# kai-neumann/OrthoSfM

Hardware: AMD Instinct MI355X
Metric: image-pairs matched/sec + BA iterations/sec (N images, M tracks) at 1/2/4/8 GPU (higher is better)
Workload: dtype i8; 1 GPU; 50 orthographic images, 20000 SIFT features/img, exhaustive matching (1225 pairs, low-res gate + two-way + cross-check + lists; SURVEY 8d's unit of work: up to, not including, RANSAC-F -- the pass through RANSAC-F is `with_geometric_verification`); views=50, features_per_view=20000, pairs=1225

## Files before the change

orthosfm_amd/csrc/match_kernels.hip:

```cpp
#include <algorithm>

#include "match_kernels.h"

namespace osfm {


typedef int v4i __attribute__((ext_vector_type(4)));
typedef int v16i __attribute__((ext_vector_type(16)));


__device__ __forceinline__ int max3i(int a, int b, int c)
{
    int r;
    asm("v_max3_i32 %0, %1, %2, %3" : "=v"(r) : "v"(a), "v"(b), "v"(c));
    return r;
}
__device__ __forceinline__ int med3a(int a, int b, int c)
{
    int r;
    asm("v_med3_i32 %0, %1, %2, %3" : "=v"(r) : "v"(a), "v"(b), "v"(c));
    return r;
}

constexpr int kGroupTiles = 8;
constexpr int kPipeGroupTiles = 16;
constexpr int kPipeTileBits = 9;
constexpr int kValNone = -(1 << 28);

template <int V> struct IntC { static constexpr int value = V; };

__device__ __forceinline__ void store_colpart(ColPart *dst, const ColPart &v)
{
#ifdef OSFM_COLPART_PLAIN_STORE
    *dst = v;
#else
    __builtin_nontemporal_store(*reinterpret_cast<const unsigned long long *>(&v), reinterpret_cast<unsigned long long *>(dst));
#endif
}

template <int CH, bool MASKED, bool RAW, bool C0>
__device__ __forceinline__ void
tile_body(const MatchProblem &pd, int rb, int seg, RowPart *__restrict__ rowparts,
    ColPart *__restrict__ colparts, char *smem, const int8_t *__restrict__ zero_tile)
{
    static_assert(!C0 || RAW, "the correction-free form needs the raw row operand");
    constexpr int D = CH * 16;
    constexpr int KS = CH / 2;
    constexpr int RPB = 16 / CH;
    constexpr int TILE_BYTES = kTileCols * D;
    constexpr int CHUNKS = kTileCols * CH;
    constexpr int CPT = CHUNKS / 256;
    constexpr int BBUF_BYTES = 2 * TILE_BYTES > 16384 ? 2 * TILE_BYTES : 16384;
    constexpr int kRawShift = C0 ? kPipeTileBits : 7;
    constexpr int kCurNone = RAW ? -(1 << (30 - kRawShift)) : kKeyNone;
    static_assert(kSegCols / kTileCols <= (1 << 7), "tile index must fit the key");
    constexpr bool PIPE = C0;
    constexpr int NCHUNK = 2 * KS;
    constexpr int RPC = 16 / NCHUNK;
    constexpr int CPC = 16 / KS;

    char *bbuf = smem;
    int *corrbuf = reinterpret_cast<int *>(smem + BBUF_BYTES);
    ColPart *colbuf = reinterpret_cast<ColPart *>(smem + BBUF_BYTES + 2 * 64 * 4);
    int *rsecbuf = reinterpret_cast<int *>(smem + BBUF_BYTES + 2 * 64 * 4 + 8 * 4 * 64 * 8);

    const int n1 = pd.n1, n2 = pd.n2, n2stride = pd.n2stride;
    const int8_t *const Bbase = C0 ? pd.B_raw : pd.B;
    const int32_t *const corrBbase = pd.corrB;
    ColPart *const colout = colparts + pd.colpart_off + (int64_t)rb * pd.n2stride;
    const int tid = threadIdx.x;
    const int wave = tid >> 6, lane = tid & 63, lr = lane & 31, lh = lane >> 5;
    const int row0 = rb * kRowsPerBlock + wave * 64;
    const int gcode = wave * 2 + lh;

    const int8_t *Abase = pd.A;
    const int32_t *corrA = pd.corrA;
    int arow0 = row0;
    if (RAW) { Abase = pd.A_raw; corrA = pd.corrA_raw; }
    else if (!MASKED && rb >= pd.nrb_main) {
        Abase = pd.A_special; corrA = pd.corrA_special;
        arow0 = (rb - pd.nrb_main) * kRowsPerBlock + wave * 64;
    }
    v4i a[2][KS];
    v16i ra[2];
#pragma unroll
    for (int rf = 0; rf < 2; ++rf) {
        const int8_t *arow = Abase + (size_t)(arow0 + rf * 32 + lr) * D;
#pragma unroll
        for (int ks = 0; ks < KS; ++ks)
            a[rf][ks] = *reinterpret_cast<const v4i *>(arow + (ks * 2 + lh) * 16);
#pragma unroll
        for (int r = 0; r < 16; ++r)
            ra[rf][r] = C0 ? 0 : corrA[arow0 + rf * 32 + (r & 3) + 8 * (r >> 2) + 4 * lh];
    }
    const v16i zero16 = {0, 0, 0, 0, 0, 0, 0, 0, 0, 0, 0, 0, 0, 0, 0, 0};
    unsigned row_valid_bits = 0xffffffffu;
    if (MASKED) {
        row_valid_bits = 0;
#pragma unroll
        for (int fr = 0; fr < 32; ++fr) {
            const int row = row0 + (fr >> 4) * 32 + (fr & 3) + 8 * ((fr >> 2) & 3) + 4 * lh;
            row_valid_bits |= (row < n1 ? 1u : 0u) << fr;
        }
    }

    v16i rbest[2], rcur[2];
#pragma unroll
    for (int rf = 0; rf < 2; ++rf)
#pragma unroll
        for (int r = 0; r < 16; ++r) {
            rbest[rf][r] = kKeyNone; rcur[rf][r] = kCurNone;
            rsecbuf[(rf * 16 + r) * 256 + tid] = kKeyNone;
        }

    const int seg_cols = pd.seg_cols;
    const int col_begin = seg * seg_cols;
    const int col_lim = min(n2, col_begin + seg_cols);
    const int ntiles = (col_lim - col_begin + kTileCols - 1) / kTileCols;

    typedef __attribute__((address_space(3))) void lds_void;
    typedef const __attribute__((address_space(1))) void glb_void;
    const int wave_s = __builtin_amdgcn_readfirstlane(wave);
    unsigned lane_off[CPT];
#pragma unroll
    for (int c = 0; c < CPT; ++c) {
        const int q = (c * 4 + wave) * 64 + lane;
        const int col = q / CH;
        const int ch = (q % CH) ^ ((col / RPB) % CH);
        lane_off[c] = (unsigned)(col * D + ch * 16);
    }
    auto dma_wait = [&](bool store_behind = false) {
        if (!PIPE) return;
#ifndef OSFM_TILE_WAIT_ALL
        if (store_behind) { asm volatile("s_waitcnt vmcnt(1)" ::: "memory"); return; }
#endif
        asm volatile("s_waitcnt vmcnt(0)" ::: "memory");
    };
    auto stage_tile = [&](int t, int buf) {
        const int8_t *src = Bbase + (size_t)(col_begin + t * kTileCols) * D;
        if (PIPE && t >= ntiles) src = zero_tile;
#pragma unroll
        for (int c = 0; c < CPT; ++c) {
            const int q0 = (c * 4 + wave_s) * 64;
            if (PIPE) {
                static_assert(!PIPE || RAW, "the PIPE schedule must not contain compiler-managed m0 users");
                const unsigned lds_at = (unsigned)(uintptr_t)(bbuf + buf * TILE_BYTES + q0 * 16);
                asm volatile("s_mov_b32 m0, %2\n\tglobal_load_lds_dwordx4 %0, %1"
                             :: "v"(lane_off[c]), "s"(src), "s"(lds_at) : "memory");
            } else {
                __builtin_amdgcn_global_load_lds(
                    (glb_void *)(src + lane_off[c]),
                    (lds_void *)(uintptr_t)(bbuf + buf * TILE_BYTES + q0 * 16), 16, 0, 0);
            }
        }
        if (!RAW && wave_s == 0)
            __builtin_amdgcn_global_load_lds(
                (glb_void *)(corrBbase + col_begin + t * kTileCols + lane),
                (lds_void *)(uintptr_t)(corrbuf + buf * 64), 4, 0, 0);
    };

    v4i b[2][KS];
    int cb_next[2] = {0, 0};
    auto load_b = [&](int buf, int cf) {
        const int col = cf * 32 + lr;
        const int swz = (col / RPB) % CH;
#pragma unroll
        for (int ks = 0; ks < KS; ++ks)
            b[cf][ks] = *reinterpret_cast<const v4i *>(
                bbuf + buf * TILE_BYTES + col * D + (((ks * 2 + lh) ^ swz) * 16));
        if (!RAW) cb_next[cf] = corrbuf[buf * 64 + col];
    };

    int cbj[2] = {0, 0}, cjt[2] = {0, 0};
    bool col_valid[2] = {true, true};
    int g[2] = {kValNone, kValNone};

    v16i acc0[2], acc1[2];

    auto phase = [&](auto ph_c, auto cl_c, auto mg_c, auto rs_c, v16i (&cur)[2], v16i (&nxt)[2], int buf_next,
                     int tile0, int tm) {
        constexpr int PH = decltype(ph_c)::value;
        constexpr int CL = decltype(cl_c)::value;
        constexpr int RS = decltype(rs_c)::value;
        constexpr bool MG = decltype(mg_c)::value != 0;
        constexpr int OF = PH ^ 1;
        int sv = 0;
        ColPart cpm[4];
        if (CL >= 0) sv = rsecbuf[(OF * 16 + CL) * 256 + tid];
        if (MG) {
#pragma unroll
            for (int w = 0; w < 4; ++w) cpm[w] = colbuf[((tm & 7) * 4 + w) * 64 + lane];
        }
#pragma unroll
        for (int i = 0; i < NCHUNK; ++i) {
            const int cf = i / KS, ks = i % KS;
            if (ks == 0)
                nxt[cf] = __builtin_amdgcn_mfma_i32_32x32x32_i8(a[PH ^ 1][0], b[cf][0], C0 ? zero16 : ra[PH ^ 1], 0, 0, 0);
            else
                nxt[cf] = __builtin_amdgcn_mfma_i32_32x32x32_i8(a[PH ^ 1][ks], b[cf][ks], nxt[cf], 0, 0, 0);
            if (PH == 0 && i == KS - 1) load_b(buf_next, 0);
            if (PH == 1 && i == 0) {
                __builtin_amdgcn_sched_barrier(0);
                load_b(buf_next, 1);
            }

#pragma unroll
            for (int r = i * RPC; r < (i + 1) * RPC; ++r) {
                if (RAW) {
                    if (RS >= 0 && r == RS) rcur[PH][r] = max(cur[0][r], cur[1][r]);
                    else rcur[PH][r] = max(max(rcur[PH][r], cur[0][r]), cur[1][r]);
                } else {
                    int k0 = (int)(((unsigned)cur[0][r] << 8) + (unsigned)cjt[0]);
                    int k1 = (int)(((unsigned)cur[1][r] << 8) + (unsigned)cjt[1]);
                    if (MASKED) {
                        k0 = col_valid[0] ? k0 : kKeyNone;
                        k1 = col_valid[1] ? k1 : kKeyNone;
                    }
                    rcur[PH][r] = max3i(rcur[PH][r], k0, k1);
                }
            }
            {
                int x[CPC];
#pragma unroll
                for (int j = 0; j < CPC; ++j) {
                    x[j] = cur[cf][ks * CPC + j];
                    if (MASKED) x[j] = ((row_valid_bits >> (PH * 16 + ks * CPC + j)) & 1u) ? x[j] : kValNone;
                }
                int gg;
                if (PH == 0 && ks == 0) gg = max(x[0], x[1]);
                else gg = max(max(g[cf], x[0]), x[1]);
#pragma unroll
                for (int j = 2; j < CPC; j += 2) gg = max(max(gg, x[j]), x[j + 1]);
                asm volatile("" : "+v"(gg));
                g[cf] = gg;
            }
            if (CL >= 0 && i == 2) {
                const int r = CL;
                const int gk = (int)(((unsigned)rcur[OF][r] << kRawShift) | (unsigned)tile0);
                rsecbuf[(OF * 16 + r) * 256 + tid] = med3a(rbest[OF][r], sv, gk);
                rbest[OF][r] = max(rbest[OF][r], gk);
            }
            if (MG && (i == 2 || i == 3)) {
                if (i == 2) {
                    int k1 = cpm[0].key_best, k2 = cpm[0].key_second;
#pragma unroll
                    for (int w = 1; w < 4; ++w) {
                        k2 = max(max(min(k1, cpm[w].key_best), k2), cpm[w].key_second);
                        k1 = max(k1, cpm[w].key_best);
                    }
                    cpm[0].key_best = k1; cpm[0].key_second = k2;
                } else {
                    store_colpart(colout + col_begin + tm * kTileCols + lane, cpm[0]);
                }
            }
            __builtin_amdgcn_sched_barrier(0);
        }
    };

    stage_tile(0, 0);
    stage_tile(PIPE || ntiles > 1 ? 1 : 0, 1);
    dma_wait();
    __syncthreads();
    load_b(0, 0);
    load_b(0, 1);
#pragma unroll
    for (int cf = 0; cf < 2; ++cf) {
        acc0[cf] = __builtin_amdgcn_mfma_i32_32x32x32_i8(a[0][0], b[cf][0], C0 ? zero16 : ra[0], 0, 0, 0);
#pragma unroll
        for (int ks = 1; ks < KS; ++ks)
            acc0[cf] = __builtin_amdgcn_mfma_i32_32x32x32_i8(a[0][ks], b[cf][ks], acc0[cf], 0, 0, 0);
    }
    __syncthreads();

    auto tile_top = [&](int t) {
        stage_tile(PIPE ? t + 2 : min(t + 2, ntiles - 1), t & 1);
#pragma unroll
        for (int cf = 0; cf < 2; ++cf) {
            if (!RAW) {
                cbj[cf] = cb_next[cf];
                cjt[cf] = (int)(((unsigned)cbj[cf] << 8) + (unsigned)(t * 2 + cf));
                asm volatile("" : "+v"(cjt[cf]));
            }
            col_valid[cf] = (col_begin + t * kTileCols + cf * 32 + lr) < n2;
        }
    };
    auto tile_bottom = [&](int t, bool store_behind = false) {
        int kk[2];
#pragma unroll
        for (int cf = 0; cf < 2; ++cf) {
            kk[cf] = (int)((unsigned)(g[cf] + cbj[cf]) << 8) | gcode;
            if (MASKED) kk[cf] = g[cf] < -(1 << 27) ? kKeyNone : kk[cf];
        }
        const auto sw = __builtin_amdgcn_permlane32_swap((unsigned)kk[0], (unsigned)kk[1], false, false);
        const int x0 = (int)sw[0], x1 = (int)sw[1];
        ColPart cp;
        cp.key_best = max(x0, x1);
        cp.key_second = min(x0, x1);
        colbuf[((t & 7) * 4 + wave) * 64 + lane] = cp;
        dma_wait(store_behind);
        __syncthreads();
    };
    auto close_all = [&](auto first_tile) {
        int sv[2][16];
#pragma unroll
        for (int rf = 0; rf < 2; ++rf)
#pragma unroll
            for (int r = 0; r < 16; ++r) sv[rf][r] = rsecbuf[(rf * 16 + r) * 256 + tid];
#pragma unroll
        for (int rf = 0; rf < 2; ++rf)
#pragma unroll
            for (int r = 0; r < 16; ++r) {
                const int gk = RAW ? (int)(((unsigned)rcur[rf][r] << kRawShift) | (unsigned)first_tile(rf, r)) : rcur[rf][r];
                rsecbuf[(rf * 16 + r) * 256 + tid] = med3a(rbest[rf][r], sv[rf][r], gk);
                rbest[rf][r] = max(rbest[rf][r], gk);
                rcur[rf][r] = kCurNone;
            }
    };
    auto merge_tile = [&](int tm) {
        ColPart cp[4];
#pragma unroll
        for (int w = 0; w < 4; ++w) cp[w] = colbuf[((tm & 7) * 4 + w) * 64 + lane];
        int k1 = cp[0].key_best, k2 = cp[0].key_second;
#pragma unroll
        for (int w = 1; w < 4; ++w) {
            k2 = max(max(min(k1, cp[w].key_best), k2), cp[w].key_second);
            k1 = max(k1, cp[w].key_best);
        }
        const int col = col_begin + tm * kTileCols + lane;
        if (col < n2stride) {
            ColPart out;
            out.key_best = k1;
            out.key_second = k2;
            store_colpart(colout + col, out);
        }
    };

    int t = 0;
    if (PIPE) {
        static_assert(kPipeGroupTiles == 16, "the staggered schedule closes one of 16 slots per phase");
        auto cycle_tile = [&](auto u_c, int t0) {
            constexpr int u = decltype(u_c)::value;
            const int tt = t0 + u;
            tile_top(tt);
            const int bn = (tt & 1) ^ 1;
            const int tm = max(tt - 5, 0) + wave;
            phase(IntC<0>(), IntC<u>(), IntC<(u & 3) == 1 ? 1 : 0>(), IntC<(u + 15) & 15>(), acc0, acc1, bn,
                max(tt - 16, 0), tm);
            phase(IntC<1>(), IntC<u>(), IntC<0>(), IntC<u>(), acc1, acc0, bn, max(tt - 15, 0), 0);
            tile_bottom(tt, (u & 3) == 1);
        };
        const int tcyc = (ntiles + 15) & ~15;
        for (; t < tcyc; t += 16) {
            cycle_tile(IntC<0>(), t); cycle_tile(IntC<1>(), t); cycle_tile(IntC<2>(), t); cycle_tile(IntC<3>(), t);
            cycle_tile(IntC<4>(), t); cycle_tile(IntC<5>(), t); cycle_tile(IntC<6>(), t); cycle_tile(IntC<7>(), t);
            cycle_tile(IntC<8>(), t); cycle_tile(IntC<9>(), t); cycle_tile(IntC<10>(), t); cycle_tile(IntC<11>(), t);
            cycle_tile(IntC<12>(), t); cycle_tile(IntC<13>(), t); cycle_tile(IntC<14>(), t); cycle_tile(IntC<15>(), t);
        }
        merge_tile(t - 4 + wave);
        rcur[0][15] = kCurNone;
        const int tc = t;
        close_all([&](int rf, int r) { return max(tc - (rf ? 16 : 15) + r, 0); });
    }
    const int t_tail = t;
    if (!PIPE)
    for (; t < ntiles; ++t) {
        tile_top(t);
        phase(IntC<0>(), IntC<-1>(), IntC<0>(), IntC<-1>(), acc0, acc1, (t & 1) ^ 1, 0, 0);
        phase(IntC<1>(), IntC<-1>(), IntC<0>(), IntC<-1>(), acc1, acc0, (t & 1) ^ 1, 0, 0);
        if (PIPE ? t == ntiles - 1 : ((t % kGroupTiles) == kGroupTiles - 1 || t == ntiles - 1)) {
            const int first = PIPE ? t_tail : (t / kGroupTiles) * kGroupTiles;
            close_all([&](int, int) { return first; });
        }
        tile_bottom(t);
        if ((t & 3) == 3 || t == ntiles - 1) {
            const int tm = (t & ~3) + wave;
            if (tm <= t) merge_tile(tm);
        }
    }

    RowPart *rp = rowparts + pd.rowpart_off + (int64_t)seg * ((int64_t)pd.nrb * kRowsPerBlock);
    int *bb = reinterpret_cast<int *>(smem);
    static_assert(BBUF_BYTES + 2 * 64 * 4 + 8 * 4 * 64 * 8 >= 32 * 256 * 4, "the best keys of both fragments must fit in front of rsecbuf");
    __syncthreads();
#pragma unroll
    for (int rf = 0; rf < 2; ++rf)
#pragma unroll
        for (int r = 0; r < 16; ++r) bb[(rf * 16 + r) * 256 + tid] = rbest[rf][r];
    __syncthreads();
    {
        constexpr int SH = RAW ? kRawShift : 8;
        const int r = lane & 15, h = (lane >> 4) & 1, rf = lane >> 5;
        const int base = (rf * 16 + r) * 256 + wave * 64 + h * 32;
        v4i kb[8], ks[8];
#pragma unroll
        for (int j = 0; j < 8; ++j) {
            const int jj = (j + r) & 7;
            kb[j] = *reinterpret_cast<const v4i *>(bb + base + jj * 4);
            ks[j] = *reinterpret_cast<const v4i *>(rsecbuf + base + jj * 4);
        }
        int b1 = kKeyNone, b2 = kKeyNone, smax = kKeyNone;
#pragma unroll
        for (int j = 0; j < 8; ++j)
#pragma unroll
            for (int e = 0; e < 4; ++e) {
                b2 = med3a(b1, b2, kb[j][e]);
                b1 = max(b1, kb[j][e]);
            }
#pragma unroll
        for (int j = 0; j < 8; j += 2)
#pragma unroll
            for (int e = 0; e < 4; ++e) smax = max3i(smax, ks[j][e], ks[j + 1][e]);
        unsigned hit = 0;
#pragma unroll
        for (int j = 7; j >= 0; --j)
#pragma unroll
            for (int e = 3; e >= 0; --e) hit = (hit << 1) | (kb[j][e] == b1 ? 1u : 0u);
        const unsigned rot = __builtin_amdgcn_alignbit(hit, hit, (32 - 4 * r) & 31);
        const int bl = 31 - __builtin_clz(rot | 1u);
        const int sk = max(b2, smax);
        const int row = row0 + rf * 32 + (r & 3) + 8 * (r >> 2) + 4 * h;
        RowPart out;
        out.ip_best = b1 == kKeyNone ? INT_MIN : (b1 >> SH);
        out.ip_second = sk == kKeyNone ? INT_MIN : (sk >> SH);
        out.idx_best = b1 == kKeyNone ? 0
                     : RAW ? col_begin + (b1 & ((1 << kRawShift) - 1)) * kTileCols + bl
                           : col_begin + (b1 & 255) * 32 + bl;
        out.pad = RAW ? 1 : 0;
        rp[row] = out;
    }
}

template <int CH, bool MASKED, bool RAW, bool C0>
__global__ __launch_bounds__(256, 2) void
match_tile_kernel(const MatchProblem *__restrict__ problems, int num_problems, int total_blocks,
    RowPart *__restrict__ rowparts, ColPart *__restrict__ colparts, unsigned long long *__restrict__ clock_probe,
    const int8_t *__restrict__ zero_tile)
{
    extern __shared__ __attribute__((aligned(16))) char smem[];
    const int lin = xcd_remap(blockIdx.x, total_blocks);
    int lo = 0, hi = num_problems - 1;
    while (lo < hi) {
        const int mid = (lo + hi + 1) >> 1;
        if (problems[mid].block_start <= lin) lo = mid; else hi = mid - 1;
    }
    const MatchProblem &pd = problems[lo];
    const int local = lin - pd.block_start;
    const int rb = local / pd.nseg;
    const int seg = local - rb * pd.nseg;
    if (!MASKED && (rb < pd.nrb_main) != RAW) return;
    if (RAW && (pd.c0 != 0) != C0) return;
    if (C0 && clock_probe != nullptr && (blockIdx.x & 1023) == 0) {
        const unsigned long long c0 = (unsigned long long)clock64(), w0 = (unsigned long long)wall_clock64();
        tile_body<CH, MASKED, RAW, C0>(pd, rb, seg, rowparts, colparts, smem, zero_tile);
        const unsigned long long c1 = (unsigned long long)clock64(), w1 = (unsigned long long)wall_clock64();
        if (threadIdx.x == 0) { atomicAdd(clock_probe, c1 - c0); atomicAdd(clock_probe + 1, w1 - w0); }
        return;
    }
    tile_body<CH, MASKED, RAW, C0>(pd, rb, seg, rowparts, colparts, smem, zero_tile);
}

void launch_match_tiles(int ch, bool masked, bool any_special, bool any_c0, bool any_corrected,
    const MatchProblem *d_problems, int num_problems, int total_blocks, RowPart *rowparts,
    ColPart *colparts, hipStream_t s, unsigned long long *clock_probe, const int8_t *zero_tile)
{
    if (total_blocks <= 0) return;
    const int d = ch * 16;
    const size_t lds = std::max<size_t>(2 * (size_t)kTileCols * d, 16384) + 2 * 64 * 4 + 8 * 4 * 64 * sizeof(ColPart) + 32 * 256 * 4;
    const dim3 grid(total_blocks), block(256);
#define OSFM_LAUNCH_TILES(CHV, MASKEDV, RAWV, C0V) \
    for (unsigned long long *PROBE = ((C0V) ? clock_probe : nullptr), *once_ = (unsigned long long *)1; once_; once_ = nullptr) \
    hipLaunchKernelGGL((match_tile_kernel<CHV, MASKEDV, RAWV, C0V>), grid, block, lds, s, d_problems, num_problems, total_blocks, rowparts, colparts, PROBE, zero_tile)
    if (masked) {
        if (ch == 8) OSFM_LAUNCH_TILES(8, true, false, false); else OSFM_LAUNCH_TILES(4, true, false, false);
        return;
    }
    if (any_c0) { if (ch == 8) OSFM_LAUNCH_TILES(8, false, true, true); else OSFM_LAUNCH_TILES(4, false, true, true); }
    if (any_corrected) { if (ch == 8) OSFM_LAUNCH_TILES(8, false, true, false); else OSFM_LAUNCH_TILES(4, false, true, false); }
    if (any_special) { if (ch == 8) OSFM_LAUNCH_TILES(8, false, false, false); else OSFM_LAUNCH_TILES(4, false, false, false); }
#undef OSFM_LAUNCH_TILES
}

__device__ __forceinline__ int
accept_match(int ip1, int ip2, int idx1, const LoweTable &tab)
{
    int b = max(ip1, 0), s = max(ip2, 0);
    const int idx = ip1 >= 0 ? idx1 : 0;
    int d1, d2;
    if (tab.is_signed) {
        b = min(b, 16129); s = min(s, 16129);
        d1 = 32258 - 2 * b; d2 = 32258 - 2 * s;
    } else {
        b = min(b, 65025); s = min(s, 65025);
        d1 = min(32767, 65025 - b) * 2; d2 = min(32767, 65025 - s) * 2;
    }
    if (d1 > tab.max_d1) return -1;
    if (d1 >= tab.reject_from[d2 >> 1]) return -1;
    return idx;
}

template <int CTRL, int ROW_MASK = 0xf>
__device__ __forceinline__ int dpp_mov(int v, int old)
{
    return __builtin_amdgcn_update_dpp(old, v, CTRL, ROW_MASK, 0xf, false);
}
constexpr int kDppXor1 = 0xB1;
constexpr int kDppXor2 = 0x4E;
constexpr int kDppHalfMirror = 0x141;
constexpr int kDppMirror = 0x140;
constexpr int kDppBcast15 = 0x142;
constexpr int kDppBcast31 = 0x143;

__device__ __forceinline__ int wave_max(int v)
{
    v = max(v, dpp_mov<kDppXor1>(v, INT_MIN));
    v = max(v, dpp_mov<kDppXor2>(v, INT_MIN));
    v = max(v, dpp_mov<kDppHalfMirror>(v, INT_MIN));
    v = max(v, dpp_mov<kDppMirror>(v, INT_MIN));
    v = max(v, dpp_mov<kDppBcast15, 0xa>(v, INT_MIN));
    v = max(v, dpp_mov<kDppBcast31, 0xc>(v, INT_MIN));
    return __builtin_amdgcn_readlane(v, 63);
}

template <int DIM, int DIR>
__device__ __forceinline__ void
rescan_groups(const MatchProblem &pd, const int (&q)[2], const int (&idx1)[2], const int (&code)[2],
    const int (&kind)[2], int lane, int (&idx_out)[2], int (&best_out)[2], int (&second_out)[2])
{
    constexpr int LPC = DIM / 16;
    constexpr int CPL = 64 / LPC;
    constexpr int NCAND = DIR == 0 ? 2 * kPipeGroupTiles : 32;
    constexpr int J = NCAND / CPL;
    const int c = lane % LPC, k = lane / LPC;
    const int8_t *Q = DIR == 0 ? pd.A : pd.B;
    const int8_t *Cm = DIR == 0 ? pd.B : pd.A;
    const int32_t *corrQ = DIR == 0 ? pd.corrA : pd.corrB;
    const int32_t *corrC = DIR == 0 ? pd.corrB : pd.corrA;

    int cand[2][J], corr_c[2][J], corr_q[2];
    int4 qv[2], cv[2][J];
#pragma unroll
    for (int u = 0; u < 2; ++u) {
        qv[u] = *reinterpret_cast<const int4 *>(Q + (size_t)q[u] * DIM + c * 16);
        corr_q[u] = corrQ[q[u]];
        int base0 = 0, lr = 0, rbase = 0, lh = 0;
        if (DIR == 0) {
            const int seg = idx1[u] / kSegCols, off = idx1[u] - seg * kSegCols;
            lr = off & 31;
            const int tile = off >> 6;
            base0 = seg * kSegCols + (kind[u] ? tile : (tile / kGroupTiles) * kGroupTiles) * kTileCols;
        } else {
            rbase = idx1[u] * kRowsPerBlock + (code[u] >> 1) * 64;
            lh = code[u] & 1;
        }
#pragma unroll
        for (int j = 0; j < J; ++j) {
            const int n = j * CPL + k;
            int cd;
            if (kind[u] >= 3) {
                cd = idx1[u] + (kind[u] == 3 ? 128 : 32) * n;
                if (cd >= (DIR == 0 ? pd.n2 : pd.n1)) cd = -1;
            } else if (DIR == 0) {
                cd = base0 + (n >> 1) * kTileCols + (n & 1) * 32 + lr;
                if (cd >= pd.n2 || (!kind[u] && n >= 2 * kGroupTiles)) cd = -1;
            } else {
                const int r = n & 15;
                cd = rbase + (n >> 4) * 32 + (r & 3) + 8 * (r >> 2) + 4 * lh;
                if (idx1[u] < pd.nrb_main && cd >= pd.n1) cd = -1;
            }
            cand[u][j] = cd;
        }
        if (DIR == 1 && kind[u] < 3 && idx1[u] >= pd.nrb_main) {
#pragma unroll
            for (int j = 0; j < J; ++j) {
                const int sidx = cand[u][j] - pd.nrb_main * kRowsPerBlock;
                cand[u][j] = sidx < pd.n_special ? pd.special_map[sidx] : -1;
            }
        }
    }
#pragma unroll
    for (int u = 0; u < 2; ++u) {
#pragma unroll
        for (int j = 0; j < J; ++j) {
            const int cs = max(cand[u][j], 0);
            cv[u][j] = *reinterpret_cast<const int4 *>(Cm + (size_t)cs * DIM + c * 16);
            corr_c[u][j] = corrC[cs];
        }
    }
#pragma unroll
    for (int u = 0; u < 2; ++u) {
        int kbest = INT_MIN, ksec = INT_MIN;
#pragma unroll
        for (int j = 0; j < J; ++j) {
            int acc = __builtin_amdgcn_sdot4(qv[u].x, cv[u][j].x, 0, false);
            acc = __builtin_amdgcn_sdot4(qv[u].y, cv[u][j].y, acc, false);
            acc = __builtin_amdgcn_sdot4(qv[u].z, cv[u][j].z, acc, false);
            acc = __builtin_amdgcn_sdot4(qv[u].w, cv[u][j].w, acc, false);
            acc += dpp_mov<kDppXor1>(acc, 0);
            acc += dpp_mov<kDppXor2>(acc, 0);
            if (LPC == 8) acc += dpp_mov<kDppHalfMirror>(acc, 0);
            const int key = cand[u][j] >= 0 ? (acc + corr_q[u] + corr_c[u][j]) * 32 + (j * CPL + k) : INT_MIN;
            ksec = med3a(kbest, ksec, key);
            kbest = max(kbest, key);
        }
        const int wbest = wave_max(kbest);
        const int wsec = wave_max(kbest == wbest ? ksec : kbest);
        const int pos = wbest & 31;
        int widx = 0;
#pragma unroll
        for (int j = 0; j < J; ++j)
            if ((pos / CPL) == j) widx = __builtin_amdgcn_readlane(cand[u][j], (pos % CPL) * LPC);
        idx_out[u] = max(widx, 0);
        best_out[u] = wbest >> 5;
        second_out[u] = wsec == INT_MIN ? INT_MIN : wsec >> 5;
    }
}

template <int DIM>
__device__ __forceinline__ void
scan_specials(const MatchProblem &pd, int dir, int q, int lane, int &best_out, int &second_out, int &idx_out)
{
    constexpr int LPC = DIM / 16, CPL = 64 / LPC;
    const int c = lane % LPC, k = lane / LPC;
    const int8_t *Q = dir == 0 ? pd.A : pd.B;
    const int8_t *Cm = dir == 0 ? pd.B_special : pd.A_special;
    const int32_t *corrC = dir == 0 ? pd.corrB_special : pd.corrA_special;
    const int32_t *map = dir == 0 ? pd.special_map_B : pd.special_map;
    const int ns = dir == 0 ? pd.nsB : pd.nsA;
    const int4 qv = *reinterpret_cast<const int4 *>(Q + (size_t)q * DIM + c * 16);
    const int corr_q = (dir == 0 ? pd.corrA : pd.corrB)[q];
    int kbest = INT_MIN, ksec = INT_MIN;
    for (int base = 0; base < ns; base += CPL) {
        const int slot = base + k;
        const bool live = slot < ns;
        const int4 cv = *reinterpret_cast<const int4 *>(Cm + (size_t)(live ? slot : 0) * DIM + c * 16);
        int acc = __builtin_amdgcn_sdot4(qv.x, cv.x, 0, false);
        acc = __builtin_amdgcn_sdot4(qv.y, cv.y, acc, false);
        acc = __builtin_amdgcn_sdot4(qv.z, cv.z, acc, false);
        acc = __builtin_amdgcn_sdot4(qv.w, cv.w, acc, false);
        acc += dpp_mov<kDppXor1>(acc, 0);
        acc += dpp_mov<kDppXor2>(acc, 0);
        if (LPC == 8) acc += dpp_mov<kDppHalfMirror>(acc, 0);
        const int key = live ? (acc + corr_q + corrC[live ? slot : 0]) * 512 + slot : INT_MIN;
        ksec = med3a(kbest, ksec, key);
        kbest = max(kbest, key);
    }
    const int wbest = wave_max(kbest);
    const int wsec = wave_max(kbest == wbest ? ksec : kbest);
    best_out = wbest >> 9;
    second_out = wsec == INT_MIN ? INT_MIN : wsec >> 9;
    idx_out = map[wbest & 511];
}

template <int DIM, bool SIGNED>
__global__ __launch_bounds__(128) void
match_finish_kernel(const MatchProblem *__restrict__ problems, const RowPart *__restrict__ rowparts,
    const ColPart *__restrict__ colparts, const RowPart *__restrict__ sp_parts, const int32_t *__restrict__ sp_col,
    LoweTable tab, int force_exact, ExactItem *__restrict__ exact_items, int32_t *__restrict__ exact_count, int exact_cap,
    int32_t *__restrict__ rs_count, RescoreItem *__restrict__ rs_items, int blocks_per_dir, int total_blocks)
{
    const int lin = xcd_remap(blockIdx.x, total_blocks);
    const int problem = lin / (2 * blocks_per_dir), within = lin - problem * 2 * blocks_per_dir;
    const MatchProblem &pd = problems[problem];
    const int dir = within / blocks_per_dir;
    const int block_x = within - dir * blocks_per_dir;
    const int q = block_x * blockDim.x + threadIdx.x;
    const int lane = threadIdx.x & 63;
    const int nq = dir == 0 ? pd.n1 : pd.n2;
    const int nc = dir == 0 ? pd.n2 : pd.n1;
    if ((int)(block_x * blockDim.x) >= nq) return;
    int32_t *out = dir == 0 ? pd.m12 : pd.m21;
    const bool active = q < nq;

    int ip1 = INT_MIN, ip2 = INT_MIN, idx1 = 0, code = 0, kind1 = 0;
    int sp_slot = -1;
    if (active && nc > 0 && pd.sp) {
        const int ns_mine = dir == 0 ? pd.nsA : pd.nsB;
        if (ns_mine > 0) sp_slot = (dir == 0 ? pd.special_slot : pd.special_slot_B)[q];
        if (sp_slot >= 0) {
            const int ns_pad = (ns_mine + 31) & ~31;
            const int chunk_cols = pd.sp_wide[dir] ? kSpWideChunk : kSpChunk;
            const int nchunk = (nc + chunk_cols - 1) / chunk_cols;
            const RowPart *rp0 = sp_parts + pd.sp_row_off[dir] + sp_slot;
            for (int c = 0; c < nchunk; ++c) {
                const RowPart p = rp0[(int64_t)c * ns_pad];
                ip2 = max(max(ip2, p.ip_second), min(ip1, p.ip_best));
                if (p.ip_best >= ip1 && p.ip_best != INT_MIN) { ip1 = p.ip_best; idx1 = p.idx_best; }
            }
            kind1 = pd.sp_wide[dir] ? 4 : 3;
        }
    }
    bool sp_scan = false;
    int sp_m1 = INT_MIN;
    if (active && nc > 0 && sp_slot < 0) {
        if (dir == 0) {
            const int64_t stride = (int64_t)pd.nrb * kRowsPerBlock;
            int slot = q;
            if (pd.special_slot && !pd.sp) {
                const int sidx = pd.special_slot[q];
                if (sidx >= 0) slot = pd.nrb_main * kRowsPerBlock + sidx;
            }
            constexpr int kBatch = 4;
            const RowPart *rp0 = rowparts + pd.rowpart_off + slot;
            const int nseg = pd.nseg;
            for (int s0 = 0; s0 < nseg; s0 += kBatch) {
                RowPart p[kBatch];
#pragma unroll
                for (int u = 0; u < kBatch; ++u) p[u] = rp0[(int64_t)min(s0 + u, nseg - 1) * stride];
                __builtin_amdgcn_sched_barrier(0);
#pragma unroll
                for (int u = 0; u < kBatch; ++u) {
                    const bool live = s0 + u < nseg;
                    const int pb = live ? p[u].ip_best : INT_MIN, ps = live ? p[u].ip_second : INT_MIN;
                    ip2 = max(max(ip2, ps), min(ip1, pb));
                    if (pb >= ip1 && pb != INT_MIN) { ip1 = pb; idx1 = p[u].idx_best; kind1 = p[u].pad; }
                }
            }
        } else {
            constexpr int kBatch = 8;
            const ColPart *cp0 = colparts + pd.colpart_off + q;
            const int nrb = pd.nrb;
            const int64_t stride = pd.n2stride;
            for (int rb0 = 0; rb0 < nrb; rb0 += kBatch) {
                ColPart p[kBatch];
#pragma unroll
                for (int u = 0; u < kBatch; ++u)
                {
                    const unsigned long long raw = __builtin_nontemporal_load(
                        reinterpret_cast<const unsigned long long *>(cp0 + (int64_t)min(rb0 + u, nrb - 1) * stride));
                    p[u].key_best = (int)(raw & 0xffffffffu); p[u].key_second = (int)(raw >> 32);
                }
                __builtin_amdgcn_sched_barrier(0);
#pragma unroll
                for (int u = 0; u < kBatch; ++u) {
                    const bool live = rb0 + u < nrb;
                    const int pb = (!live || p[u].key_best == kKeyNone) ? INT_MIN : (p[u].key_best >> 8);
                    const int ps = (!live || p[u].key_second == kKeyNone) ? INT_MIN : (p[u].key_second >> 8);
                    ip2 = max(max(ip2, ps), min(ip1, pb));
                    if (pb >= ip1 && pb != INT_MIN) { ip1 = pb; idx1 = rb0 + u; code = p[u].key_best & 255; }
                }
            }
        }
        if (pd.sp && (dir == 0 ? pd.nsB : pd.nsA) > 0) {
            const int t1 = sp_col[pd.sp_col_off[dir ^ 1] + q];
            if (t1 >= ip1 && t1 != INT_MIN) {
                sp_m1 = ip1; ip1 = t1; sp_scan = true;
            } else {
                ip2 = max(ip2, t1);
            }
        }
    }
    const int limit = tab.is_signed ? 32767 : 65535;
    bool exact = active && nc > 0 && (force_exact || pd.force_exact || ip1 > limit);
    bool refine = false;
    int res = -1;
    if (active && nc > 0 && !exact) {
        res = accept_match(ip1, sp_scan ? max(sp_m1, ip2) : ip2, 0, tab);
        if (res >= 0) {
            if (ip1 < 0) { res = 0; sp_scan = false; }
            else if ((sp_scan ? sp_m1 : ip2) == ip1) { exact = true; sp_scan = false; }
            else if (!sp_scan) refine = true;
        } else {
            sp_scan = false;
        }
    } else {
        sp_scan = false;
    }
    bool deferred = false;
    if (!SIGNED && DIM == 128 && rs_count != nullptr && refine) {
        int b = -1, sub = 0, cap = 0;
        int64_t item = 0;
        const int nb1 = pd.nrb_main * 4;
        if (dir == 1) {
            if (kind1 == 0 && idx1 < pd.nrb_main && code < 8) {
                b = idx1 * 4 + (code >> 1); sub = code & 1;
                item = (int64_t)b * kRescoreCap1; cap = kRescoreCap1;
            }
        } else if (kind1 == 1) {
            const int tq = idx1 >> 6;
            if (tq < (pd.n2 + kTileCols - 1) / kTileCols) {
                const int w = tq / kRescoreWin, k = w * 32 + (idx1 & 31);
                b = nb1 + k; sub = tq - w * kRescoreWin;
                item = (int64_t)nb1 * kRescoreCap1 + (int64_t)k * kRescoreCap0; cap = kRescoreCap0;
            }
        }
        if (b >= 0) {
            const int slot = atomicAdd(rs_count + pd.rs_bucket_off + b, 1);
            if (slot < cap) {
                RescoreItem it;
                it.q_sub = q * 32 + sub; it.ip2 = ip2;
                rs_items[pd.rs_item_off + item + slot] = it;
                refine = false; deferred = true;
            }
        }
    }
    unsigned long long todo = __ballot(refine);
    int rbest = 0, rsecond = 0, ridx = 0;
    while (todo) {
        int src[2], qs[2], is[2], cs[2], ks[2], idx[2], found[2], second[2];
        src[0] = __ffsll((long long)todo) - 1;
        todo &= todo - 1;
        src[1] = todo ? __ffsll((long long)todo) - 1 : src[0];
        todo &= todo - 1;
#pragma unroll
        for (int u = 0; u < 2; ++u) {
            qs[u] = __builtin_amdgcn_readlane(q, src[u]);
            is[u] = __builtin_amdgcn_readlane(idx1, src[u]);
            cs[u] = __builtin_amdgcn_readlane(code, src[u]);
            ks[u] = __builtin_amdgcn_readlane(kind1, src[u]);
        }
        if (dir == 0) rescan_groups<DIM, 0>(pd, qs, is, cs, ks, lane, idx, found, second);
        else rescan_groups<DIM, 1>(pd, qs, is, cs, ks, lane, idx, found, second);
#pragma unroll
        for (int u = 0; u < 2; ++u)
            if (lane == src[u]) { rbest = found[u]; rsecond = second[u]; ridx = idx[u]; }
    }
    if (refine) {
        rsecond = max(rsecond, ip2);
        res = accept_match(rbest, rsecond, ridx, tab);
        if (res >= 0 && rsecond == rbest) exact = true;
    }
    unsigned long long todo2 = __ballot(sp_scan);
    while (todo2) {
        const int src = __ffsll((long long)todo2) - 1;
        todo2 &= todo2 - 1;
        const int qs = __builtin_amdgcn_readlane(q, src);
        int wb, ws, wi;
        scan_specials<DIM>(pd, dir, qs, lane, wb, ws, wi);
        if (lane == src) { rbest = wb; rsecond = ws; ridx = wi; }
    }
    if (sp_scan) {
        rsecond = max(max(rsecond, sp_m1), ip2);
        res = accept_match(rbest, rsecond, ridx, tab);
        if (res >= 0 && rsecond == rbest) exact = true;
    }
    if (exact) {
        const int slot = atomicAdd(exact_count, 1);
        if (slot < exact_cap) {
            ExactItem it;
            it.problem = problem; it.dir = dir; it.query = q;
            exact_items[slot] = it;
        }
    }
    if (active && !deferred) out[q] = res;
}

void launch_match_finish(const MatchProblem *d_problems, int num_problems, int max_n,
    const RowPart *rowparts, const ColPart *colparts, const RowPart *sp_parts, const int32_t *sp_col, LoweTable tab, int force_exact,
    ExactItem *exact_items, int32_t *exact_count, int exact_cap, int32_t *rs_count, RescoreItem *rs_items, hipStream_t s)
{
    if (num_problems <= 0 || max_n <= 0) return;
    const int blocks_per_dir = (max_n + 127) / 128;
    const int64_t total = (int64_t)blocks_per_dir * 2 * num_problems;
    if (total > INT_MAX) return;
    const dim3 grid((unsigned)total);
    if (tab.is_signed)
        hipLaunchKernelGGL((match_finish_kernel<64, true>), grid, dim3(128), 0, s, d_problems, rowparts,
            colparts, sp_parts, sp_col, tab, force_exact, exact_items, exact_count, exact_cap, nullptr, nullptr,
            blocks_per_dir, (int)total);
    else
        hipLaunchKernelGGL((match_finish_kernel<128, false>), grid, dim3(128), 0, s, d_problems, rowparts,
            colparts, sp_parts, sp_col, tab, force_exact, exact_items, exact_count, exact_cap, rs_count, rs_items,
            blocks_per_dir, (int)total);
}

constexpr int kRescorePerWave = 16;
static_assert(2 * (kRescoreWin + 15) <= 64, "a direction-0 bucket's candidates fill two MFMA blocks at most");

__global__ __launch_bounds__(256, 4) void
match_rescore_kernel(const MatchProblem *__restrict__ problems, int num_problems, const int32_t *__restrict__ rs_count,
    const RescoreItem *__restrict__ rs_items, int total_buckets, int total_blocks, LoweTable tab,
    ExactItem *__restrict__ exact_items, int32_t *__restrict__ exact_count, int exact_cap)
{
    __shared__ __attribute__((aligned(16))) int corr_s[4][64];
    const int lin = xcd_remap(blockIdx.x, total_blocks);
    const int wv = threadIdx.x >> 6, lane = threadIdx.x & 63, h = lane >> 5, j = lane & 31;
    const int b0 = (lin * 4 + wv) * kRescorePerWave;
    if (b0 >= total_buckets) return;
    const int cnt_l = lane < kRescorePerWave && b0 + lane < total_buckets ? rs_count[b0 + lane] : 0;
    unsigned long long todo = __ballot(cnt_l > 0);
    if (!todo) return;
    int p = 0;
    {
        const int b = b0 + __ffsll((long long)todo) - 1;
        int lo = 0, hi = num_problems - 1;
        while (lo < hi) {
            const int mid = (lo + hi + 1) >> 1;
            if (problems[mid].rs_bucket_off <= b) lo = mid; else hi = mid - 1;
        }
        p = lo;
    }
    const v16i zero16 = {0, 0, 0, 0, 0, 0, 0, 0, 0, 0, 0, 0, 0, 0, 0, 0};
    while (todo) {
        const int k = __ffsll((long long)todo) - 1;
        todo &= todo - 1;
        const int b = b0 + k;
        while (p + 1 < num_problems && problems[p + 1].rs_bucket_off <= b) ++p;
        const MatchProblem &pd = problems[p];
        const int local = b - (int)pd.rs_bucket_off;
        const int nb1 = pd.nrb_main * 4;
        const int dir = local < nb1 ? 1 : 0;
        int strip = 0, w0 = 0, lr = 0, cap;
        int64_t item0;
        if (dir == 1) {
            strip = (local >> 2) * kRowsPerBlock + (local & 3) * 64;
            cap = kRescoreCap1;
            item0 = pd.rs_item_off + (int64_t)local * kRescoreCap1;
        } else {
            const int l0 = local - nb1;
            w0 = (l0 >> 5) * kRescoreWin; lr = l0 & 31;
            cap = kRescoreCap0;
            item0 = pd.rs_item_off + (int64_t)nb1 * kRescoreCap1 + (int64_t)l0 * kRescoreCap0;
        }
        auto cand_of = [&](int o) {
            if (dir == 1) { const int r = strip + o; return r < pd.n1 ? r : -1; }
            const int c = kTileCols * (w0 + (o >> 1)) + 32 * (o & 1) + lr;
            return c < pd.n2 ? c : -1;
        };
        const int cnt = min(__builtin_amdgcn_readlane(cnt_l, k), cap);
        const int8_t *Cm = dir == 0 ? pd.B : pd.A;
        const int8_t *Qm = dir == 0 ? pd.A : pd.B;
        const int32_t *corrC = dir == 0 ? pd.corrB : pd.corrA;
        const int32_t *corrQ = dir == 0 ? pd.corrA : pd.corrB;
        int32_t *out = dir == 0 ? pd.m12 : pd.m21;
        RescoreItem it0;
        it0.q_sub = 0; it0.ip2 = 0;
        if (j < cnt) it0 = rs_items[item0 + j];
        v4i a[2][4];
#pragma unroll
        for (int bk = 0; bk < 2; ++bk) {
            const int cs = max(cand_of(32 * bk + j), 0);
#pragma unroll
            for (int ks = 0; ks < 4; ++ks)
                a[bk][ks] = *reinterpret_cast<const v4i *>(Cm + (size_t)cs * 128 + (ks * 2 + h) * 16);
        }
        {
            const int c = cand_of(lane);
            corr_s[wv][lane] = c >= 0 ? corrC[c] : INT_MIN;
        }
        __builtin_amdgcn_wave_barrier();
        for (int qb = 0; qb < cnt; qb += 32) {
            const bool live = qb + j < cnt;
            RescoreItem it = it0;
            if (qb > 0) {
                it.q_sub = 0; it.ip2 = 0;
                if (live) it = rs_items[item0 + qb + j];
            }
            const int q = it.q_sub >> 5, sub = it.q_sub & 31;
            v4i bq[4];
#pragma unroll
            for (int ks = 0; ks < 4; ++ks)
                bq[ks] = *reinterpret_cast<const v4i *>(Qm + (size_t)q * 128 + (ks * 2 + h) * 16);
            const int cq = corrQ[q];
            v16i acc[2];
#pragma unroll
            for (int bk = 0; bk < 2; ++bk) {
                acc[bk] = __builtin_amdgcn_mfma_i32_32x32x32_i8(a[bk][0], bq[0], zero16, 0, 0, 0);
#pragma unroll
                for (int ks = 1; ks < 4; ++ks)
                    acc[bk] = __builtin_amdgcn_mfma_i32_32x32x32_i8(a[bk][ks], bq[ks], acc[bk], 0, 0, 0);
            }
            int kbest = INT_MIN, ksec = INT_MIN;
#pragma unroll
            for (int bk = 0; bk < 2; ++bk)
#pragma unroll
                for (int g = 0; g < 4; ++g) {
                    const int ob = 32 * bk + 8 * g + 4 * h;
                    const v4i cc = *reinterpret_cast<const v4i *>(&corr_s[wv][ob]);
#pragma unroll
                    for (int e = 0; e < 4; ++e) {
                        const int o = ob + e;
                        int n;
                        bool ok;
                        if (dir == 1) {
                            n = 16 * bk + 4 * g + e;
                            ok = h == sub;
                        } else {
                            n = o - 2 * sub;
                            ok = (unsigned)n < 32u;
                        }
                        const int key = ok && cc[e] != INT_MIN ? (acc[bk][4 * g + e] + cq + cc[e]) * 32 + n : INT_MIN;
                        ksec = med3a(kbest, ksec, key);
                        kbest = max(kbest, key);
                    }
                }
            const int obest = __shfl_xor(kbest, 32), osec = __shfl_xor(ksec, 32);
            const int wbest = max(kbest, obest);
            const int wsec = max(min(kbest, obest), max(ksec, osec));
            if (live && h == 0) {
                const int pos = wbest & 31;
                const int o = dir == 1 ? 32 * (pos >> 4) + (pos & 3) + 8 * ((pos >> 2) & 3) + 4 * sub : pos + 2 * sub;
                const int idx = max(cand_of(o), 0);
                const int rbest = wbest >> 5;
                const int rsecond = max(wsec == INT_MIN ? INT_MIN : wsec >> 5, it.ip2);
                const int res = accept_match(rbest, rsecond, idx, tab);
                out[q] = res;
                if (res >= 0 && rsecond == rbest) {
                    const int slot = atomicAdd(exact_count, 1);
                    if (slot < exact_cap) {
                        ExactItem e;
                        e.problem = p; e.dir = dir; e.query = q;
                        exact_items[slot] = e;
                    }
                }
            }
        }
        __builtin_amdgcn_wave_barrier();
    }
}

void launch_match_rescore(const MatchProblem *d_problems, int num_problems, const int32_t *rs_count,
    const RescoreItem *rs_items, int64_t total_buckets, LoweTable tab, ExactItem *exact_items, int32_t *exact_count,
    int exact_cap, hipStream_t s)
{
    if (num_problems <= 0 || total_buckets <= 0) return;
    const int64_t blocks = (total_buckets + 4 * kRescorePerWave - 1) / (4 * kRescorePerWave);
    if (total_buckets > INT_MAX || blocks > INT_MAX) return;
    hipLaunchKernelGGL(match_rescore_kernel, dim3((unsigned)blocks), dim3(256), 0, s, d_problems, num_problems,
        rs_count, rs_items, (int)total_buckets, (int)blocks, tab, exact_items, exact_count, exact_cap);
}

template <int DIM, bool SIGNED>
__global__ __launch_bounds__(256) void
exact_scan_kernel(const MatchProblem *__restrict__ problems, const ExactItem *__restrict__ items,
    const int32_t *__restrict__ count, int exact_cap, LoweTable tab)
{
    const int lane = threadIdx.x & 63;
    const int wave_global = (blockIdx.x * blockDim.x + threadIdx.x) >> 6;
    const int nwaves = (gridDim.x * blockDim.x) >> 6;
    const int n_items = min(*count, exact_cap);
    for (int it = wave_global; it < n_items; it += nwaves) {
        const ExactItem item = items[it];
        const MatchProblem &pd = problems[item.problem];
        const int8_t *Q = item.dir == 0 ? pd.A : pd.B;
        const int8_t *C = item.dir == 0 ? pd.B : pd.A;
        const int nc = item.dir == 0 ? pd.n2 : pd.n1;
        int32_t *out = item.dir == 0 ? pd.m12 : pd.m21;
        const int8_t *qrow = Q + (size_t)item.query * DIM;
        int best = 0, second = 0, idx = 0;
        for (int base = 0; base < nc; base += 64) {
            const int j = base + lane;
            int ip = 0;
            if (j < nc) {
// ... 302 lines not shown
```

Baseline: 21700 pairs/s.

## Split column partials into separate best/second planes to cut finish-kernel reads

Column partial results are stored as two separate int32 planes (best keys, then second keys) instead of interleaved 64-bit pairs, using scalar-base nontemporal dword stores in the pipelined path. The finish kernel then reads only the best-key plane across row blocks and fetches a single second-key from the winning block, roughly halving the bytes it scans; the batch size rises to 16. The producer now issues two stores per column, so the DMA wait threshold changes to vmcnt(2), and correctness relies on the second-best of non-winning blocks never exceeding their best.

```diff
diff --git a/orthosfm_amd/csrc/match_kernels.hip b/orthosfm_amd/csrc/match_kernels.hip
--- a/orthosfm_amd/csrc/match_kernels.hip
+++ b/orthosfm_amd/csrc/match_kernels.hip
@@ -29,13 +29,21 @@
 
 template <int V> struct IntC { static constexpr int value = V; };
 
-__device__ __forceinline__ void store_colpart(ColPart *dst, const ColPart &v)
-{
+__device__ __forceinline__ void store_colpart(int32_t *best, int32_t *second, unsigned byte_off, const ColPart &v)
+{
+    int32_t *const pb = reinterpret_cast<int32_t *>(reinterpret_cast<char *>(best) + byte_off);
+    int32_t *const ps = reinterpret_cast<int32_t *>(reinterpret_cast<char *>(second) + byte_off);
 #ifdef OSFM_COLPART_PLAIN_STORE
-    *dst = v;
+    *pb = v.key_best; *ps = v.key_second;
 #else
-    __builtin_nontemporal_store(*reinterpret_cast<const unsigned long long *>(&v), reinterpret_cast<unsigned long long *>(dst));
+    __builtin_nontemporal_store(v.key_best, pb);
+    __builtin_nontemporal_store(v.key_second, ps);
 #endif
+}
+__device__ __forceinline__ void store_colpart_sbase(int32_t *best, int32_t *second, unsigned byte_off, const ColPart &v)
+{
+    asm volatile("global_store_dword %0, %1, %2 nt" :: "v"(byte_off), "v"(v.key_best), "s"(best) : "memory");
+    asm volatile("global_store_dword %0, %1, %2 nt" :: "v"(byte_off), "v"(v.key_second), "s"(second) : "memory");
 }
 
 template <int CH, bool MASKED, bool RAW, bool C0>
@@ -67,7 +75,8 @@
     const int n1 = pd.n1, n2 = pd.n2, n2stride = pd.n2stride;
     const int8_t *const Bbase = C0 ? pd.B_raw : pd.B;
     const int32_t *const corrBbase = pd.corrB;
-    ColPart *const colout = colparts + pd.colpart_off + (int64_t)rb * pd.n2stride;
+    int32_t *const colbest = reinterpret_cast<int32_t *>(colparts + pd.colpart_off) + (int64_t)rb * pd.n2stride;
+    int32_t *const colsecond = colbest + (int64_t)pd.nrb * pd.n2stride;
     const int tid = threadIdx.x;
     const int wave = tid >> 6, lane = tid & 63, lr = lane & 31, lh = lane >> 5;
     const int row0 = rb * kRowsPerBlock + wave * 64;
@@ -121,6 +130,8 @@
     typedef __attribute__((address_space(3))) void lds_void;
     typedef const __attribute__((address_space(1))) void glb_void;
     const int wave_s = __builtin_amdgcn_readfirstlane(wave);
+    unsigned lane4 = (unsigned)lane * 4u;
+    if (PIPE) asm volatile("" : "+v"(lane4));
     unsigned lane_off[CPT];
 #pragma unroll
     for (int c = 0; c < CPT; ++c) {
@@ -132,7 +143,7 @@
     auto dma_wait = [&](bool store_behind = false) {
         if (!PIPE) return;
 #ifndef OSFM_TILE_WAIT_ALL
-        if (store_behind) { asm volatile("s_waitcnt vmcnt(1)" ::: "memory"); return; }
+        if (store_behind) { asm volatile("s_waitcnt vmcnt(2)" ::: "memory"); return; }
 #endif
         asm volatile("s_waitcnt vmcnt(0)" ::: "memory");
     };
@@ -178,7 +189,7 @@
     v16i acc0[2], acc1[2];
 
     auto phase = [&](auto ph_c, auto cl_c, auto mg_c, auto rs_c, v16i (&cur)[2], v16i (&nxt)[2], int buf_next,
-                     int tile0, int tm) {
+                     int tile0, int tm, int tms) {
         constexpr int PH = decltype(ph_c)::value;
         constexpr int CL = decltype(cl_c)::value;
         constexpr int RS = decltype(rs_c)::value;
@@ -250,7 +261,7 @@
                     }
                     cpm[0].key_best = k1; cpm[0].key_second = k2;
                 } else {
-                    store_colpart(colout + col_begin + tm * kTileCols + lane, cpm[0]);
+                    store_colpart_sbase(colbest + col_begin + tms * kTileCols, colsecond + col_begin + tms * kTileCols, lane4, cpm[0]);
                 }
             }
             __builtin_amdgcn_sched_barrier(0);
@@ -331,7 +342,7 @@
             ColPart out;
             out.key_best = k1;
             out.key_second = k2;
-            store_colpart(colout + col, out);
+            store_colpart(colbest, colsecond, (unsigned)col * 4u, out);
         }
     };
 
@@ -345,8 +356,8 @@
             const int bn = (tt & 1) ^ 1;
             const int tm = max(tt - 5, 0) + wave;
             phase(IntC<0>(), IntC<u>(), IntC<(u & 3) == 1 ? 1 : 0>(), IntC<(u + 15) & 15>(), acc0, acc1, bn,
-                max(tt - 16, 0), tm);
-            phase(IntC<1>(), IntC<u>(), IntC<0>(), IntC<u>(), acc1, acc0, bn, max(tt - 15, 0), 0);
+                max(tt - 16, 0), tm, max(tt - 5, 0) + wave_s);
+            phase(IntC<1>(), IntC<u>(), IntC<0>(), IntC<u>(), acc1, acc0, bn, max(tt - 15, 0), 0, 0);
             tile_bottom(tt, (u & 3) == 1);
         };
         const int tcyc = (ntiles + 15) & ~15;
@@ -365,8 +376,8 @@
     if (!PIPE)
     for (; t < ntiles; ++t) {
         tile_top(t);
-        phase(IntC<0>(), IntC<-1>(), IntC<0>(), IntC<-1>(), acc0, acc1, (t & 1) ^ 1, 0, 0);
-        phase(IntC<1>(), IntC<-1>(), IntC<0>(), IntC<-1>(), acc1, acc0, (t & 1) ^ 1, 0, 0);
+        phase(IntC<0>(), IntC<-1>(), IntC<0>(), IntC<-1>(), acc0, acc1, (t & 1) ^ 1, 0, 0, 0);
+        phase(IntC<1>(), IntC<-1>(), IntC<0>(), IntC<-1>(), acc1, acc0, (t & 1) ^ 1, 0, 0, 0);
         if (PIPE ? t == ntiles - 1 : ((t % kGroupTiles) == kGroupTiles - 1 || t == ntiles - 1)) {
             const int first = PIPE ? t_tail : (t / kGroupTiles) * kGroupTiles;
             close_all([&](int, int) { return first; });
@@ -651,6 +662,10 @@
     idx_out = map[wbest & 511];
 }
 
+#ifndef OSFM_FINISH_BATCH
+#define OSFM_FINISH_BATCH 16
+#endif
+
 template <int DIM, bool SIGNED>
 __global__ __launch_bounds__(128) void
 match_finish_kernel(const MatchProblem *__restrict__ problems, const RowPart *__restrict__ rowparts,
@@ -716,28 +731,27 @@
                 }
             }
         } else {
-            constexpr int kBatch = 8;
-            const ColPart *cp0 = colparts + pd.colpart_off + q;
+            constexpr int kBatch = OSFM_FINISH_BATCH;
+            const int32_t *best0 = reinterpret_cast<const int32_t *>(colparts + pd.colpart_off) + q;
             const int nrb = pd.nrb;
             const int64_t stride = pd.n2stride;
             for (int rb0 = 0; rb0 < nrb; rb0 += kBatch) {
-                ColPart p[kBatch];
+                int kb[kBatch];
 #pragma unroll
                 for (int u = 0; u < kBatch; ++u)
-                {
-                    const unsigned long long raw = __builtin_nontemporal_load(
-                        reinterpret_cast<const unsigned long long *>(cp0 + (int64_t)min(rb0 + u, nrb - 1) * stride));
-                    p[u].key_best = (int)(raw & 0xffffffffu); p[u].key_second = (int)(raw >> 32);
-                }
+                    kb[u] = __builtin_nontemporal_load(best0 + (int64_t)min(rb0 + u, nrb - 1) * stride);
                 __builtin_amdgcn_sched_barrier(0);
 #pragma unroll
                 for (int u = 0; u < kBatch; ++u) {
                     const bool live = rb0 + u < nrb;
-                    const int pb = (!live || p[u].key_best == kKeyNone) ? INT_MIN : (p[u].key_best >> 8);
-                    const int ps = (!live || p[u].key_second == kKeyNone) ? INT_MIN : (p[u].key_second >> 8);
-                    ip2 = max(max(ip2, ps), min(ip1, pb));
-                    if (pb >= ip1 && pb != INT_MIN) { ip1 = pb; idx1 = rb0 + u; code = p[u].key_best & 255; }
+                    const int pb = (!live || kb[u] == kKeyNone) ? INT_MIN : (kb[u] >> 8);
+                    ip2 = max(ip2, min(ip1, pb));
+                    if (pb >= ip1 && pb != INT_MIN) { ip1 = pb; idx1 = rb0 + u; code = kb[u] & 255; }
                 }
+            }
+            if (ip1 != INT_MIN) {
+                const int ks = __builtin_nontemporal_load(best0 + ((int64_t)nrb + idx1) * stride);
+                ip2 = max(ip2, ks == kKeyNone ? INT_MIN : (ks >> 8));
             }
         }
         if (pd.sp && (dir == 0 ? pd.nsB : pd.nsA) > 0) {
```

Result: faster. 22100 pairs/s, median of 6 (+1.8%).
